# teshnizi/GraphEnvs

Measured on AMD Instinct MI355X. Metric: env-steps/sec (whole node), ShortestPath-v0 n=64 m=192 batch=65536, 1/2/4/8 GPU, higher is better.
Workload: dtype u64; 1 GPU; ShortestPath-v0 n_nodes=64 n_edges=192 weighted, 65536 env slots per GPU, random valid actions on device, same-step autoreset (seed-exact G(n,m)+features on device); envs_per_gpu=65536, prefetch_period=0, episodes_finished_per_gpu=6165512, settle_steps=128, parallelism=batch shard x1, no collective

## Files before the change

graphenvs_amd/csrc/ge_reset.h:

```cpp
#pragma once
#include "ge_params.h"
#include "ge_platform.h"

GE_DEV double ge_wlut(int code) {
  const int k = (code >= 3 && code <= 9) ? code : 10;
  return (double)k / 10.0;
}

GE_DEV uint32_t ge_temper(uint32_t y) {
  y ^= (y >> 11);
  y ^= (y << 7) & 0x9d2c5680u;
  y ^= (y << 15) & 0xefc60000u;
  y ^= (y >> 18);
  return y;
}

GE_DEV void ge_mt_twist(uint32_t *mt, int lane) {
  const int lo[3] = {0, GE_MT_N - GE_MT_M, 2 * (GE_MT_N - GE_MT_M)}, hi[3] = {GE_MT_N - GE_MT_M, 2 * (GE_MT_N - GE_MT_M), GE_MT_N};
#pragma unroll
  for (int ph = 0; ph < 3; ph++) {
    uint32_t a[4], b[4], c[4];
#pragma unroll
    for (int k = 0; k < 4; k++) {
      const int i = lo[ph] + lane + 64 * k;
// ... 89 lines not shown
  ge_wave_sync();
}


GE_DEV void ge_mt_load(uint32_t *mt, const uint32_t *src, int lane) {
  uint32_t r[10];
#pragma unroll
  for (int k = 0; k < 10; k++) { int i = lane + 64 * k; r[k] = i < GE_MT_N ? src[i] : 0u; }
#pragma unroll
  for (int k = 0; k < 10; k++) { int i = lane + 64 * k; if (i < GE_MT_N) mt[i] = r[k]; }
  ge_wave_sync();
}

GE_DEV void ge_mt_save(uint32_t *dst, const uint32_t *mt, int pos, int lane) {
  ge_wave_sync();
#pragma unroll
  for (int k = 0; k < 10; k++) { int i = lane + 64 * k; if (i < GE_MT_N) dst[i] = mt[i]; }
  if (lane == 0) dst[GE_MT_N] = (uint32_t)pos;
}

GE_DEV int ge_wave_incl_scan(int x, int lane) {
  for (int off = 1; off < GE_WAVE; off <<= 1) {
    int t = ge_shfl_i32(x, lane >= off ? lane - off : 0);
    if (lane >= off) x += t;
  }
  return x;
}

GE_DEV uint32_t ge_mask_below(uint32_t v) {
  return v ? (0xffffffffu >> ge_clz32(v)) : 0u;
}

struct GeRctx {
  uint32_t *mt, *mt2, *wm; uint64_t *abits; uint32_t *elist; int *fill; int *rowptr; uint16_t *colw; uint8_t *wsort;
  uint32_t *tmp; int *dist; int *perm;
  double *sigma, *delta;
  uint64_t *bits; int *misc;
};

GE_DEV GeRctx ge_carve(const GeParams &P) {
  unsigned char *s = ge_dyn_smem();
  const GeLds &L = P.lds;
  GeRctx c;
  c.mt = (uint32_t *)(s + L.mt); c.mt2 = (uint32_t *)(s + L.mt2); c.wm = (uint32_t *)(s + L.wm); c.abits = (uint64_t *)(s + L.abits); c.elist = (uint32_t *)(s + L.elist);
  c.fill = (int *)(s + L.fill); c.rowptr = (int *)(s + L.rowptr); c.colw = (uint16_t *)(s + L.colw);
  c.wsort = (uint8_t *)(s + L.wsort); c.tmp = (uint32_t *)(s + L.tmp); c.dist = (int *)(s + L.dist);
  c.perm = (int *)(s + L.perm);
  double *f = (double *)(s + L.f64a);
  c.sigma = f; c.delta = f + P.n;
  c.bits = (uint64_t *)(s + L.bits); c.misc = (int *)(s + L.misc);
  return c;
}

GE_DEV int ge_reach_wave(const GeRctx &c, int ng, int W, int start, const uint64_t *removed, int lane) {
  uint64_t *fr = c.bits, *vis = c.bits + W, *nx = c.bits + 2 * W;
  if (lane < W) {
    uint64_t s = ((start >> 6) == lane) ? (1ull << (start & 63)) : 0ull;
    fr[lane] = s; vis[lane] = s | (removed ? removed[lane] : 0ull);
  }
  ge_wave_sync();
  for (;;) {
    uint64_t any = 0;
    for (int k = 0; k < W; k++) {
      int v = k * GE_WAVE + lane;
      bool hit = false;
      if (v < ng && !((vis[k] >> lane) & 1ull)) {
        for (int w = 0; w < W; w++) if (c.abits[v * W + w] & fr[w]) { hit = true; break; }
      }
      uint64_t b = ge_ballot(hit);
      if (lane == 0) nx[k] = b;
      any |= b;
    }
    ge_wave_sync();
    if (!any) break;
    if (lane < W) { vis[lane] |= nx[lane]; fr[lane] = nx[lane]; }
    ge_wave_sync();
  }
  int cnt = 0;
  for (int w = 0; w < W; w++) cnt += ge_popc64(vis[w] & ~(removed ? removed[w] : 0ull));
  ge_wave_sync();
  return cnt;
}

GE_DEV bool ge_connected(const GeRctx &c, int ng, int W, int skip, int lane) {
  uint64_t *rem = c.bits + 3 * W;
  if (lane < W) rem[lane] = (skip >= 0 && (skip >> 6) == lane) ? (1ull << (skip & 63)) : 0ull;
  ge_wave_sync();
  int start = (skip == 0) ? 1 : 0;
  return ge_reach_wave(c, ng, W, start, rem, lane) == ng - (skip >= 0 ? 1 : 0);
}

GE_DEV double ge_pw_leaf(const double *a, int n, int lane) {
  if (n < 8) {
    double res = 0.0;
    for (int i = 0; i < n; i++) res += a[i];
    return res;
  }
  int lim = n - (n % 8);
  double r = 0.0;
  if (lane < 8) { r = a[lane]; for (int i = 8; i < lim; i += 8) r += a[i + lane]; }
  double r0 = ge_shfl_f64(r, 0), r1 = ge_shfl_f64(r, 1), r2 = ge_shfl_f64(r, 2), r3 = ge_shfl_f64(r, 3);
  double r4 = ge_shfl_f64(r, 4), r5 = ge_shfl_f64(r, 5), r6 = ge_shfl_f64(r, 6), r7 = ge_shfl_f64(r, 7);
  double res = ((r0 + r1) + (r2 + r3)) + ((r4 + r5) + (r6 + r7));
  for (int i = lim; i < n; i++) res += a[i];
  return res;
}
template <int D>
GE_DEV double ge_pw(const double *a, int n, int lane) {
  if (n <= 128) return ge_pw_leaf(a, n, lane);
  if constexpr (D > 0) {
    int n2 = n / 2; n2 -= n2 % 8;
    double l = ge_pw<D - 1>(a, n2, lane);
    double r = ge_pw<D - 1>(a + n2, n - n2, lane);
    return l + r;
  } else {
    return 0.0;
  }
}

GE_DEV int ge_rank_below(const uint64_t *row, int v) {
  int r = 0;
  for (int w = 0; w < (v >> 6); w++) r += ge_popc64(row[w]);
  return r + ge_popc64(row[v >> 6] & ((1ull << (v & 63)) - 1ull));
}

GE_DEV int ge_list_nbr(const GeParams &P, const GeRctx &c, int idx) {
  if (P.nocolw) { const int u = (int)(((uint64_t)(uint32_t)idx * P.div_m) >> 40), k = idx - u * (P.ng - 1); return k < u ? k : k + 1; }
  return (int)(c.colw[idx] >> 4);
}
GE_DEV int ge_list_code(const GeParams &P, const GeRctx &c, int idx) {
  if (P.nowsort) {
    if (!P.weighted) return 10;
    const int u = (int)(((uint64_t)(uint32_t)idx * P.div_m) >> 40), k = idx - u * (P.ng - 1), v = k < u ? k : k + 1;
    const int a = u < v ? u : v, b = u < v ? v : u;
    return (int)((const uint8_t *)c.wm)[a * (P.ng - 1) - ((a * (a - 1)) >> 1) + (b - a - 1)];
  }
  return P.nocolw ? (int)c.wsort[idx] : (int)(c.colw[idx] & 15);
}

GE_DEV int ge_row_of(const GeParams &P, const GeRctx &c, int idx) {
  return P.complete ? (int)(((uint64_t)(uint32_t)idx * P.div_m) >> 40) : (int)c.tmp[idx];
}

GE_DEV int ge_sorted_pos(const GeRctx &c, int W, int u, int v) { return c.rowptr[u] + ge_rank_below(c.abits + u * W, v); }
GE_DEV int ge_sorted_pos_p(const GeParams &P, const GeRctx &c, int u, int v) {
  return P.complete ? c.rowptr[u] + v - (v > u ? 1 : 0) : ge_sorted_pos(c, P.W, u, v);
}


struct GeInject { const int64_t *links; const uint8_t *wcode; const float *x; const int32_t *terminals; const uint32_t *seeds; };
#ifndef GE_GNM_ROUND_CAP
#define GE_GNM_ROUND_CAP (1 << 22)
#endif


#if defined(GE_STAMPS) && !defined(GE_EMU)
__device__ unsigned long long ge_stamp_buf[32];
#define GE_STAMP(k) do { if (lane == 0 && env == 0) { ge_stamp_buf[k] = wall_clock64(); if ((k) == 11) ge_stamp_buf[30] = clock64(); if ((k) == 17) ge_stamp_buf[31] = clock64(); } } while (0)
#define GE_STAMP_T0(k) do { if (tid == 0 && env == 0) ge_stamp_buf[k] = wall_clock64(); } while (0)
#define GE_STAMP_B0(k) do { if (lane == 0 && ge_bid() == 0) ge_stamp_buf[k] = wall_clock64(); } while (0)
#elif defined(GE_STAMP_SLOTS) && !defined(GE_EMU)
#define GE_STAMP(k) do { if (lane == 0) { if ((k) == 0) P.buf.final_cost[env] = (double)wall_clock64(); else if ((k) == 2) P.buf.final_len[env] = (int32_t)(wall_clock64() - (unsigned long long)P.buf.final_cost[env]); else if ((k) == 10) P.buf.final_heur[env] = (double)wall_clock64(); } } while (0)
#define GE_STAMP_T0(k) do { } while (0)
#define GE_STAMP_B0(k) do { } while (0)
#else
#define GE_STAMP(k) do { } while (0)
#define GE_STAMP_T0(k) do { } while (0)
#define GE_STAMP_B0(k) do { } while (0)
#endif


GE_DEV void ge_np_sink(const GeParams &P, const GeRctx &c, int sink, int idx, uint32_t val) {
  const int n = P.n, W = P.W;
  const uint32_t code = (sink == 3 ? 1u : 3u) + val;
  if (sink == 3) ((uint8_t *)c.wm)[P.cost_off + idx] = (uint8_t)code;
  else if (sink == 0) atomicOr(&c.wm[idx >> 3], code << (4 * (idx & 7)));
  else if (sink == 1) ((uint8_t *)c.wm)[idx] = (uint8_t)code;
  else {
    const int i = (int)((unsigned)idx / (unsigned)n), j = idx - i * n;
    if (i < j && ((c.abits[i * W + (j >> 6)] >> (j & 63)) & 1ull)) {
      c.wsort[ge_sorted_pos(c, W, i, j)] = (uint8_t)code; c.wsort[ge_sorted_pos(c, W, j, i)] = (uint8_t)code;
    }
  }
}

GE_DEV void ge_np_draws(const GeParams &P, const GeRctx &c, uint32_t *mt, int &nppos, int total, int lane, int sink) {
  int base = 0;
  const uint32_t bm = (sink == 3) ? 3u : 7u;
  const uint64_t below = (1ull << lane) - 1ull;
  while (base < total) {
    if (nppos >= GE_MT_N && total - base > GE_MT_N) {
      uint32_t R[GE_MT_ROWS];
      ge_mt_to_regs(R, mt, lane);
      do {
        ge_mt_twist_regs(R, lane);
#pragma unroll
        for (int k = 0; k < GE_MT_ROWS; k++) {
          const uint32_t val = (GE_WAVE * k + lane < GE_MT_N) ? (ge_temper(R[k]) & bm) : bm;
          const uint64_t bal = ge_ballot(val < bm);
          if (val < bm) ge_np_sink(P, c, sink, base + ge_popc64(bal & below), val);
          base += ge_popc64(bal);
        }
      } while (total - base > GE_MT_N);
      ge_mt_from_regs(mt, R, lane);
      ge_wave_sync();
      nppos = GE_MT_N;
      continue;
    }
    if (nppos >= GE_MT_N) { ge_mt_twist(mt, lane); nppos = 0; }
    if (GE_MT_N - nppos >= 4 * GE_WAVE) {
      uint32_t val[4]; uint64_t bal[4];
#pragma unroll
      for (int k = 0; k < 4; k++) val[k] = ge_temper(mt[nppos + GE_WAVE * k + lane]) & bm;
      int tot = 0;
#pragma unroll
      for (int k = 0; k < 4; k++) { bal[k] = ge_ballot(val[k] < bm); tot += ge_popc64(bal[k]); }
      if (base + tot < total) {
        int off = base;
#pragma unroll
        for (int k = 0; k < 4; k++) {
          if (val[k] < bm) ge_np_sink(P, c, sink, off + ge_popc64(bal[k] & below), val[k]);
          off += ge_popc64(bal[k]);
        }
        base = off; nppos += 4 * GE_WAVE;
        continue;
      }
    }
    {
      const int p = nppos + lane; const bool valid = p < GE_MT_N;
      const uint32_t val = valid ? (ge_temper(mt[p]) & bm) : 8u;
      const bool acc = valid && val < bm;
      const uint64_t bal = ge_ballot(acc);
      const int rank = ge_popc64(bal & below);
      const int idx = base + rank;
      if (acc && idx < total) ge_np_sink(P, c, sink, idx, val);
      const int nacc = ge_popc64(bal);
      if (base + nacc >= total) {
        const int need = total - base - 1;
        const uint64_t lastb = ge_ballot(acc && rank == need);
        nppos += ge_ctz64(lastb) + 1;
        base = total;
      } else {
        base += nacc;
        nppos += (GE_MT_N - nppos < GE_WAVE) ? (GE_MT_N - nppos) : GE_WAVE;
      }
    }
  }
  ge_wave_sync();
}

GE_DEV void ge_np_edge_cells(const GeParams &P, const GeRctx &c, uint32_t *tcell, int lane) {
  const int n = P.n, W = P.W;
  {
    int carry = 0;
    for (int k0 = 0; k0 < n; k0 += GE_WAVE) {
      const int u = k0 + lane; int d = 0;
      if (u < n) for (int w = u >> 6; w < W; w++) { uint64_t b = c.abits[u * W + w]; if (w == (u >> 6)) b &= ~((2ull << (u & 63)) - 1ull); d += ge_popc64(b); }
      const int incl = ge_wave_incl_scan(d, lane);
      if (u < n) c.dist[u] = carry + incl - d;
      carry += ge_shfl_i32(incl, GE_WAVE - 1);
    }
    ge_wave_sync();
    for (int u = lane; u < n; u += GE_WAVE) {
      int t = c.dist[u];
      for (int w = u >> 6; w < W; w++) {
        uint64_t b = c.abits[u * W + w]; if (w == (u >> 6)) b &= ~((2ull << (u & 63)) - 1ull);
        for (; b; b &= b - 1) tcell[t++] = (uint32_t)(u * n + w * 64 + ge_ctz64(b));
      }
    }
    ge_wave_sync();
  }
}
GE_DEV int ge_np_edge_number(const GeRctx &c, int W, int u, int v) {
  const int a = u < v ? u : v, b = u < v ? v : u;
  int t = c.dist[a];
  for (int w = a >> 6; w <= (b >> 6); w++) {
    uint64_t bits = c.abits[a * W + w];
    if (w == (a >> 6)) bits &= ~((2ull << (a & 63)) - 1ull);
    if (w == (b >> 6)) bits &= (1ull << (b & 63)) - 1ull;
    t += ge_popc64(bits);
  }
  return t;
}
GE_DEV void ge_np_draws_cells(const GeParams &P, const GeRctx &c, uint32_t *mt, int &nppos, int lane, const uint32_t *tcell, uint8_t *tcode) {
  const int n = P.n, m = P.m, total = n * n;
  const uint64_t below = (1ull << lane) - 1ull;
  GE_STAMP_B0(7);
  int base = 0, t = 0, t0 = 0;
  uint32_t treg = lane < m ? tcell[lane] : 0xffffffffu;
  uint32_t next = ge_readlane_u32(treg, 0);
  auto take = [&](uint32_t val, uint64_t bal, int cnt) {
    while (next - (uint32_t)base < (uint32_t)cnt) {
      const int r = (int)(next - (uint32_t)base);
      if (((bal >> lane) & 1ull) && ge_popc64(bal & below) == r) tcode[t] = (uint8_t)(3u + val);
      t++;
      if (t - t0 == GE_WAVE) { t0 = t; treg = (t0 + lane < m) ? tcell[t0 + lane] : 0xffffffffu; }
      next = ge_readlane_u32(treg, t - t0);
    }
  };
  while (base < total) {
    if (nppos >= GE_MT_N && total - base > GE_MT_N) {
      uint32_t R[GE_MT_ROWS];
      ge_mt_to_regs(R, mt, lane);
      do {
        ge_mt_twist_regs(R, lane);
        int tot = 0;
// ... 692 lines not shown
    if (path_like) {
      for (int i = lane; i < (n * n + 7) / 8; i += GE_WAVE) c.wm[i] = 0u;
      ge_wave_sync();
      ge_np_draws(P, c, c.mt2, nppos, n * n, lane, 0);
    } else ge_np_draws(P, c, c.mt2, nppos, t == GE_TSP ? P.m : n, lane, 1);
  }
  GE_STAMP(22);
  if (t == GE_DISTRIBUTION_CENTER) ge_np_draws(P, c, c.mt2, nppos, n, lane, 3);
  if (t == GE_PERISHABLE_DELIVERY) {
    const uint32_t ra = ge_np_next(c.mt2, nppos, lane), rb = ge_np_next(c.mt2, nppos, lane);
    if (lane == 0) { *(double *)c.misc = ((double)(int32_t)(ra >> 5) * 67108864.0 + (double)(int32_t)(rb >> 6)) / 9007199254740992.0; c.misc[2] = nppos; }
    ge_wave_sync();
    return;
  }
  if (t == GE_MULTICAST_ROUTING) ge_np_multicast_tail(P, c, c.mt2, nppos, lane);
  else if (path_like) ge_np_terminals(P, c, c.mt2, nppos, lane, n, P.T);
  GE_STAMP(23);
  if (save) ge_mt_save(save, c.mt2, nppos, lane);
}

template <class RP, class CW>
GE_DEV uint64_t ge_dc_search(double cutoff, int n, int s, const RP *rowptr, const CW *colw, double *S, int ss, uint8_t *stk, int ks) {
  (void)stk; (void)ks;
  for (int v = 0; v < n; v++) S[v * ss] = __builtin_inf();
  S[s * ss] = 0.0;
  uint64_t reached = 1ull << s, cur = 1ull << s;
  while (cur) {
    uint64_t nxt = 0;
    for (; cur; cur &= cur - 1) {
      const int u = ge_ctz64(cur);
      const double du = S[u * ss];
      const int r1 = rowptr[u + 1];
      for (int k0 = rowptr[u]; k0 < r1; k0 += 4) {
        uint32_t e[4]; double sv[4];
#pragma unroll
        for (int j = 0; j < 4; j++) e[j] = (uint32_t)colw[k0 + j < r1 ? k0 + j : k0];
#pragma unroll
        for (int j = 0; j < 4; j++) sv[j] = S[(int)(e[j] >> 4) * ss];
#pragma unroll
        for (int j = 0; j < 4; j++) {
          const int v = (int)(e[j] >> 4);
          const double d = du + ge_wlut((int)(e[j] & 15u));
          if (k0 + j < r1 && d <= cutoff && d < sv[j]) {
            S[v * ss] = d; reached |= 1ull << v;
            if (d + 0.3 <= cutoff) nxt |= 1ull << v;
          }
        }
      }
    }
    cur = nxt;
  }
  return reached;
}

template <int ENV>
GE_DEV void ge_write_edge_slabs(const GeParams &P, const GeRctx &c, int env, int tid, int nthreads) {
  constexpr int t = ENV;
  const ge_buffers &G = P.buf;
  const int n = P.n, W = P.W, E = P.E;
  const int64_t nbase = (int64_t)env * n, ebase = (int64_t)env * E, Ne = P.edge_row_stride;
  for (int idx = tid; idx < E; idx += nthreads) {
    int u = ge_row_of(P, c, idx), v = ge_list_nbr(P, c, idx), code = ge_list_code(P, c, idx);
    G.edge_index[ebase + idx] = P.node_id_base + nbase + u;
    G.edge_index[Ne + ebase + idx] = P.node_id_base + nbase + v;
    float wv = (t == GE_DENSEST_SUBGRAPH || t == GE_MAX_INDEPENDENT_SET) ? 1.f : (float)ge_wlut(code);
    if (P.spatial) wv = (float)G.sw64[ebase + ge_sorted_pos_p(P, c, u, v)];
    if (P.Fe == 2) { G.edge_attr[(ebase + idx) * 2] = wv; G.edge_attr[(ebase + idx) * 2 + 1] = 0.f; }
    else G.edge_attr[ebase + idx] = wv;
    G.colw[ebase + idx] = (uint16_t)((v << 4) | code);
    G.scode[ebase + idx] = P.nowsort ? (uint8_t)code : c.wsort[idx];
    if (G.rev_edge) {
      const int r0 = c.rowptr[v], r1 = c.rowptr[v + 1];
      int r = -1;
      for (int k0 = r0; k0 < r1 && r < 0; k0 += 4) {
        int w[4];
#pragma unroll
        for (int j = 0; j < 4; j++) w[j] = (int)(c.colw[k0 + j < r1 ? k0 + j : r0] >> 4);
#pragma unroll
        for (int j = 3; j >= 0; j--) if (k0 + j < r1 && w[j] == u) r = k0 + j;
      }
      G.rev_edge[ebase + idx] = r;
    }
  }
  for (int v = tid; v <= n; v += nthreads) G.row_ptr[(int64_t)env * (n + 1) + v] = c.rowptr[v];
  for (int i = tid; i < n * W; i += nthreads) G.adj_bits[nbase * W + i] = c.abits[i];
  if (G.node_rec) {
    for (int v = tid; v < n; v += nthreads) {
      uint64_t codes = 0; int d = c.rowptr[v + 1] - c.rowptr[v]; if (d > 16) d = 16;
      for (int k = 0; k < d; k++) codes |= (uint64_t)(c.wsort[c.rowptr[v] + k] & 15) << (4 * k);
      G.node_rec[(nbase + v) * 2] = c.abits[v]; G.node_rec[(nbase + v) * 2 + 1] = codes;
    }
  }
}

template <int ENV>
GE_DEV void ge_reset_env(const GeParams &P, int env, const uint32_t *seeds, const GeRun &run, const GeInject &inj) {
  const int tid = ge_tid_fresh();
  const int lane = tid & (GE_WAVE - 1);
  const int wv = tid >> 6;
  const int n = P.n, ng = P.ng, W = P.W, m = P.m, E = P.E, F = P.F, T = P.T;
  constexpr int t = ENV;
  const bool path_like_t = (t == GE_SHORTEST_PATH || t == GE_LONGEST_PATH || t == GE_STEINER_TREE || t == GE_MULTICAST_ROUTING);
  GeRctx c = ge_carve(P);
  const int64_t nbase = (int64_t)env * n, ebase = (int64_t)env * E;
  const bool restart = run.restart != 0;
  const bool next = run.next != 0;
  const bool queued = run.items == GE_ITEMS_QUEUE && !run.refill;
  const int64_t episode = restart ? 0 : P.buf.episode[env] + (next ? 1 : 0);
  const uint32_t seed = restart ? (run.restart == 1 ? seeds[env] : inj.seeds[env]) : P.buf.seed[env] + (next ? (uint32_t)P.seed_stride : 0u);
  const int ring = (int)(episode % GE_SEED_DEPTH);
  auto keep_at = [&](int which) -> uint32_t * { return P.buf.stream_state ? P.buf.stream_state + ((int64_t)env * 2 + which) * GE_STREAM_WORDS : nullptr; };
  auto pos0 = [&](int which) -> int { return run.cont ? (int)keep_at(which)[GE_MT_N] : GE_MT_N; };
  const uint32_t *mt_src = P.buf.mt_state + ((int64_t)env * GE_SEED_DEPTH + ring) * 2 * GE_MT_N;
  if (run.cont) mt_src = keep_at(0);
  int src = 0, dest = -1;
  int ppd_pk[5] = {-1, -1, -1, -1, -1}, ppd_dp[5] = {-1, -1, -1, -1, -1};
  bool gen_failed = false;
  double ppd_dt = 0.0;
  if (wv == 1) {
    if (!run.inject) { ge_numpy_wave<ENV>(P, c, run.cont ? keep_at(1) : mt_src + GE_MT_N, lane, env, pos0(1), keep_at(1)); ge_sync(); }
    ge_sync();
    ge_write_edge_slabs<ENV>(P, c, env, tid, 2 * GE_WAVE);
    ge_sync();
    return;
  }

  GE_STAMP(0);
  if (!run.inject) {
    ge_mt_load(c.mt, mt_src, lane);
    GE_STAMP(1);
    int pypos = pos0(0);
    int ppd_attempt = 0, ppd_pos = 0;
    bool failed = false;
    const int shift = 32 - (32 - ge_clz32((uint32_t)ng));
    for (;;) {
      GE_STAMP(29);
      for (int i = lane; i < n * W; i += GE_WAVE) c.abits[i] = 0ull;
      ge_wave_sync();
      if (P.complete) {
        for (int v = lane; v < ng; v += GE_WAVE)
          for (int w = 0; w < W; w++) {
            int lo = w * 64, hi = lo + 64; if (hi > ng) hi = ng;
            uint64_t bitsw = (hi <= lo) ? 0ull : ((hi - lo == 64) ? ~0ull : ((1ull << (hi - lo)) - 1ull));
            if ((v >> 6) == w) bitsw &= ~(1ull << (v & 63));
            c.abits[v * W + w] = bitsw;
          }
      } else {
        int cnt = 0, have_u = 0, carry_u = 0;
        const uint64_t below = (1ull << lane) - 1ull;
        int rounds = 0;
        for (;;) {
          if (++rounds > GE_GNM_ROUND_CAP) { failed = true; break; }
          if (pypos >= GE_MT_N) { ge_mt_twist(c.mt, lane); pypos = 0; }
          const int p0 = pypos + lane, p1 = p0 + GE_WAVE;
          const bool valid0 = p0 < GE_MT_N, valid1 = p1 < GE_MT_N;
          const uint32_t r0 = valid0 ? (ge_temper(c.mt[p0]) >> shift) : (uint32_t)ng, r1 = valid1 ? (ge_temper(c.mt[p1]) >> shift) : (uint32_t)ng;
          const bool pick0 = valid0 && r0 < (uint32_t)ng, pick1 = valid1 && r1 < (uint32_t)ng;
          const uint64_t V0 = ge_ballot(pick0), V1 = ge_ballot(pick1);
          const int n0 = ge_popc64(V0);
          const bool is_v0 = pick0 && ((ge_popc64(V0 & below) + have_u) & 1), is_v1 = pick1 && ((n0 + ge_popc64(V1 & below) + have_u) & 1);
          const uint64_t b0 = V0 & below, b1 = V1 & below;
          const uint32_t ur0 = ge_shfl_u32(r0, b0 ? 63 - (int)__builtin_clzll(b0) : 0), ur1 = ge_shfl_u32(r1, b1 ? 63 - (int)__builtin_clzll(b1) : 0);
          const int last0 = V0 ? (int)ge_readlane_u32(r0, 63 - (int)__builtin_clzll(V0)) : carry_u;
          const int u0 = b0 ? (int)ur0 : carry_u, v0 = (int)r0, u1 = b1 ? (int)ur1 : last0, v1 = (int)r1;
          const bool elig0 = is_v0 && u0 != v0 && !((c.abits[u0 * W + (v0 >> 6)] >> (v0 & 63)) & 1ull);
          const bool elig1 = is_v1 && u1 != v1 && !((c.abits[u1 * W + (v1 >> 6)] >> (v1 & 63)) & 1ull);
          const uint32_t key0 = elig0 ? (uint32_t)((u0 < v0 ? u0 : v0) << 12 | (u0 < v0 ? v0 : u0)) : 0xffffffffu;
          const uint32_t key1 = elig1 ? (uint32_t)((u1 < v1 ? u1 : v1) << 12 | (u1 < v1 ? v1 : u1)) : 0xfffffffeu;
          (void)ge_ballot(elig0 || elig1);
          bool lost0 = false, lost1 = false;
          if (elig0) {
            const int a = u0 < v0 ? u0 : v0, b = u0 < v0 ? v0 : u0; const unsigned long long bit = 1ull << (b & 63);
            lost0 = (atomicOr((unsigned long long *)&c.abits[a * W + (b >> 6)], bit) & bit) != 0;
          }
          if (elig1) {
            const int a = u1 < v1 ? u1 : v1, b = u1 < v1 ? v1 : u1; const unsigned long long bit = 1ull << (b & 63);
            lost1 = (atomicOr((unsigned long long *)&c.abits[a * W + (b >> 6)], bit) & bit) != 0;
          }
          bool dup0 = false, dup1 = false;
          uint64_t rem0 = ge_ballot(lost0), rem1 = ge_ballot(lost1);
          while (rem0 | rem1) {
            const uint32_t k0 = rem0 ? ge_readlane_u32(key0, ge_ctz64(rem0)) : ge_readlane_u32(key1, ge_ctz64(rem1));
            const uint64_t same0 = ge_ballot(elig0 && key0 == k0), same1 = ge_ballot(elig1 && key1 == k0);
            if (elig0 && key0 == k0 && lane != ge_ctz64(same0)) dup0 = true;
            if (elig1 && key1 == k0 && (same0 != 0ull || lane != ge_ctz64(same1))) dup1 = true;
            rem0 &= ~same0; rem1 &= ~same1;
          }
          bool acc0 = elig0 && !dup0, acc1 = elig1 && !dup1;
          const uint64_t A0 = ge_ballot(acc0), A1 = ge_ballot(acc1);
          const int na0 = ge_popc64(A0), na1 = ge_popc64(A1);
          const int arank0 = ge_popc64(A0 & below), arank1 = na0 + ge_popc64(A1 & below);
          const bool last_round = cnt + na0 + na1 >= m;
          int consumed, nacc = na0 + na1;
          if (last_round) {
            const int need = m - cnt - 1;
            bool undo0 = false, undo1 = false;
            if (need < na0) { const int fl = ge_ctz64(ge_ballot(acc0 && arank0 == need)); undo0 = acc0 && lane > fl; undo1 = acc1; acc0 = acc0 && lane <= fl; acc1 = false; consumed = fl + 1; }
            else { const int fl = ge_ctz64(ge_ballot(acc1 && arank1 == need)); undo1 = acc1 && lane > fl; acc1 = acc1 && lane <= fl; consumed = GE_WAVE + fl + 1; }
            if (undo0) { const int a = u0 < v0 ? u0 : v0, b = u0 < v0 ? v0 : u0; atomicAnd((unsigned long long *)&c.abits[a * W + (b >> 6)], ~(1ull << (b & 63))); }
            if (undo1) { const int a = u1 < v1 ? u1 : v1, b = u1 < v1 ? v1 : u1; atomicAnd((unsigned long long *)&c.abits[a * W + (b >> 6)], ~(1ull << (b & 63))); }
            nacc = need + 1;
          } else {
            consumed = (GE_MT_N - pypos < 2 * GE_WAVE) ? (GE_MT_N - pypos) : 2 * GE_WAVE;
            const int npick = n0 + ge_popc64(V1) + have_u;
            have_u = npick & 1;
            if (have_u && (V0 | V1)) carry_u = V1 ? (int)ge_readlane_u32(r1, 63 - (int)__builtin_clzll(V1)) : last0;
          }
          if (acc0) {
            atomicOr((unsigned long long *)&c.abits[u0 * W + (v0 >> 6)], (unsigned long long)(1ull << (v0 & 63)));
            atomicOr((unsigned long long *)&c.abits[v0 * W + (u0 >> 6)], (unsigned long long)(1ull << (u0 & 63)));
            c.elist[cnt + arank0] = (uint32_t)u0 | ((uint32_t)v0 << 16);
          }
          if (acc1) {
            atomicOr((unsigned long long *)&c.abits[u1 * W + (v1 >> 6)], (unsigned long long)(1ull << (v1 & 63)));
            atomicOr((unsigned long long *)&c.abits[v1 * W + (u1 >> 6)], (unsigned long long)(1ull << (u1 & 63)));
            c.elist[cnt + arank1] = (uint32_t)u1 | ((uint32_t)v1 << 16);
          }
          cnt += nacc; pypos += consumed;
          ge_wave_sync();
          if (last_round) break;
        }
      }
      ge_wave_sync();
      GE_STAMP(26);
      if (failed) break;
      uint64_t low = 0;
      for (int k = 0; k < W; k++) {
        const int v = k * GE_WAVE + lane; int d = 0;
        if (v < ng) for (int w = 0; w < W; w++) d += ge_popc64(c.abits[v * W + w]);
        low |= ge_ballot(v < ng && (d == 0 || (t == GE_TSP && d == 1)));
      }
      GE_STAMP(27);
      bool ok = !low && ge_connected(c, ng, W, -1, lane);
      GE_STAMP(28);
      if (ok && t == GE_TSP) ok = ge_connected(c, ng, W, 0, lane);
      if (ok && t == GE_PERISHABLE_DELIVERY) {
        double rnd;
        const bool late = P.weighted && !P.np_early;
        if (ppd_attempt == 0) { ge_sync(); if (late) ppd_pos = pos0(1); else { ppd_pos = c.misc[2]; rnd = *(const double *)c.misc; } }
        if (ppd_attempt > 0 || late) {
          if (late) { ge_np_edge_cells(P, c, c.tmp, lane); ge_np_draws_cells(P, c, c.mt2, ppd_pos, lane, c.tmp, (uint8_t *)c.wm); }
          else if (P.weighted) { for (int i = lane; i < (n * n + 7) / 8; i += GE_WAVE) c.wm[i] = 0u; ge_wave_sync(); ge_np_draws(P, c, c.mt2, ppd_pos, n * n, lane, 0); }
          const uint32_t ra = ge_np_next(c.mt2, ppd_pos, lane), rb = ge_np_next(c.mt2, ppd_pos, lane);
          rnd = ((double)(int32_t)(ra >> 5) * 67108864.0 + (double)(int32_t)(rb >> 6)) / 9007199254740992.0;
        }
        ppd_attempt++;
        ok = (n > GE_PPD_WIDE_ABOVE) ? ge_ppd_place_wide(P, c, rnd, ppd_pos, ppd_pk, ppd_dp, ppd_dt, lane)
                       : ge_ppd_place(P, c, (double *)(ge_dyn_smem() + P.lds.fw), rnd, ppd_pos, ppd_pk, ppd_dp, ppd_dt, lane);
      }
      if (ok) break;
      ge_wave_priority(1);
    }
    ge_wave_priority(0);
    if (failed) {
      if (lane == 0) atomicOr((unsigned int *)&P.buf.work_count[1], 1u);
      gen_failed = true;
      for (int i = lane; i < n * W; i += GE_WAVE) c.abits[i] = 0ull;
      ge_wave_sync();
      if (lane == 0) {
        int cnt = 0;
        for (int d = 1; d < ng && cnt < m; d++)
          for (int u = 0; u + d < ng && cnt < m; u++) {
            const int v = u + d;
            c.abits[u * W + (v >> 6)] |= 1ull << (v & 63); c.abits[v * W + (u >> 6)] |= 1ull << (u & 63);
            c.elist[cnt++] = (uint32_t)u | ((uint32_t)v << 16);
          }
      }
      ge_wave_sync();
      if (t == GE_PERISHABLE_DELIVERY) { if (ppd_attempt == 0) { ge_sync(); ppd_pos = c.misc[2]; } for (int i = 0; i < P.n_dests; i++) { ppd_pk[i] = i; ppd_dp[i] = P.n_dests + i; } }
    }
    if (P.buf.stream_state) {
      ge_mt_save(keep_at(0), c.mt, pypos, lane);
      if (t == GE_PERISHABLE_DELIVERY) ge_mt_save(keep_at(1), c.mt2, ppd_pos, lane);
    }
  } else {
    for (int i = lane; i < n * W; i += GE_WAVE) c.abits[i] = 0ull;
    for (int v = lane; v < n; v += GE_WAVE) c.fill[v] = 0;
    ge_wave_sync();
    for (int idx = lane; idx < E; idx += GE_WAVE) {
      int u = (int)inj.links[(ebase + idx) * 2], v = (int)inj.links[(ebase + idx) * 2 + 1];
      atomicAdd(&c.fill[u], 1);
      atomicOr((unsigned long long *)&c.abits[u * W + (v >> 6)], (unsigned long long)(1ull << (v & 63)));
    }
    ge_wave_sync();
  }

  GE_STAMP(2);
  if (!run.inject) {
    for (int v = lane; v < n; v += GE_WAVE) { int d = 0; for (int w = 0; w < W; w++) d += ge_popc64(c.abits[v * W + w]); c.fill[v] = d; }
    ge_wave_sync();
  }
  {
    int carry = 0;
    for (int k0 = 0; k0 < n; k0 += GE_WAVE) {
      int v = k0 + lane; int d = v < n ? c.fill[v] : 0;
      int incl = ge_wave_incl_scan(d, lane);
      if (v < n) c.rowptr[v] = carry + incl - d;
      carry += ge_shfl_i32(incl, GE_WAVE - 1);
    }
    if (lane == 0) c.rowptr[n] = carry;
    ge_wave_sync();
  }
  if (run.inject) {
    for (int idx = lane; idx < E; idx += GE_WAVE) {
      int u = (int)inj.links[(ebase + idx) * 2], v = (int)inj.links[(ebase + idx) * 2 + 1];
      c.colw[idx] = (uint16_t)((v << 4) | (inj.wcode[ebase + idx] & 15));
      if (!P.complete) c.tmp[idx] = (uint32_t)u;
    }
    ge_wave_sync();
  } else if (P.complete) {
    if (!P.nocolw) for (int idx = lane; idx < E; idx += GE_WAVE) {
      const int u = ge_row_of(P, c, idx), k = idx - u * (ng - 1);
      int v = k < u ? k : k + 1;
      c.colw[idx] = (uint16_t)((v << 4) | 10);
    }
    ge_wave_sync();
  } else {
    for (int v = lane; v < n; v += GE_WAVE) c.fill[v] = 0;
    ge_wave_sync();
    for (int id = lane; id < m; id += GE_WAVE) {
      uint32_t e = c.elist[id]; int u = (int)(e & 0xffffu), v = (int)(e >> 16);
      int s = c.rowptr[u] + atomicAdd(&c.fill[u], 1); c.tmp[s] = ((uint32_t)id << 16) | (uint32_t)v;
      int s2 = c.rowptr[v] + atomicAdd(&c.fill[v], 1); c.tmp[s2] = ((uint32_t)id << 16) | (uint32_t)u;
    }
    ge_wave_sync();
    for (int v = lane; v < n; v += GE_WAVE) {
      int lo = c.rowptr[v], hi = c.rowptr[v + 1];
      for (int a = lo + 1; a < hi; a++) {
        uint32_t key = c.tmp[a]; int b = a - 1;
        while (b >= lo && c.tmp[b] > key) { c.tmp[b + 1] = c.tmp[b]; b--; }
        c.tmp[b + 1] = key;
      }
    }
    ge_wave_sync();
    for (int idx = lane; idx < E; idx += GE_WAVE) c.colw[idx] = (uint16_t)(((c.tmp[idx] & 0xffffu) << 4) | 10u);
    ge_wave_sync();
    for (int v = lane; v < n; v += GE_WAVE) for (int k = c.rowptr[v]; k < c.rowptr[v + 1]; k++) c.tmp[k] = (uint32_t)v;
    ge_wave_sync();
  }

  GE_STAMP(3);
  if (!run.inject && t != GE_PERISHABLE_DELIVERY) ge_sync();
  if (!run.inject) {
    if (!P.nowsort) for (int idx = lane; idx < E; idx += GE_WAVE) c.wsort[idx] = 10;
    ge_wave_sync();
    const bool path_like = path_like_t;
    const bool matrix_w = path_like_t || t == GE_DISTRIBUTION_CENTER || t == GE_PERISHABLE_DELIVERY;
    if (P.weighted && matrix_w && P.np_early) {
      for (int idx = lane; idx < E; idx += GE_WAVE) {
        int u = ge_row_of(P, c, idx), v = c.colw[idx] >> 4;
        int a = u < v ? u : v, b = u < v ? v : u, cell = a * n + b;
        c.wsort[ge_sorted_pos_p(P, c, u, v)] = (uint8_t)((c.wm[cell >> 3] >> (4 * (cell & 7))) & 15u);
      }
    } else if (P.spatial) {
      const double *xy = (const double *)(c.wm + 4 * n);
      for (int idx = lane; idx < E; idx += GE_WAVE) {
        int u = ge_row_of(P, c, idx), v = c.colw[idx] >> 4;
        int a = u < v ? u : v, b = u < v ? v : u;
        double dx = xy[2 * a] - xy[2 * b], dy = xy[2 * a + 1] - xy[2 * b + 1];
        P.buf.sw64[ebase + ge_sorted_pos_p(P, c, u, v)] = __builtin_sqrt(dx * dx + dy * dy);
      }
    } else if (P.weighted && t == GE_TSP && P.complete) {
      if (!P.nowsort) for (int idx = lane; idx < E; idx += GE_WAVE) {
        const int u = ge_row_of(P, c, idx), v = ge_list_nbr(P, c, idx);
        const int a = u < v ? u : v, b = u < v ? v : u;
        c.wsort[ge_sorted_pos_p(P, c, u, v)] = ((const uint8_t *)c.wm)[a * (ng - 1) - ((a * (a - 1)) >> 1) + (b - a - 1)];
      }
    } else if (P.weighted && t == GE_TSP) {
      int carry = 0;
// ... 447 lines not shown
```

Measured before the change: 396.2 million env-steps/s.

## Compact picked MT samples into one pair per lane in G(n,m) edge sampling

The G(n,m) edge sampler now reads four wave-widths of Mersenne Twister output per round, ballots which samples fall in range, and compacts them so each lane handles one (u,v) pair, located through a popcount-based select64. Before, each lane tested two raw slots, and only about half the picked samples became the v of a pair. The goal is to fill the wave with candidate edges each round, so fewer rounds and fewer duplicate-resolution ballots are needed. The cost is extra select/popcount work and gathered mt reads per round, plus more intricate consumed/carry bookkeeping that must keep the seed-exact sequence.

```diff
diff --git a/graphenvs_amd/csrc/ge_reset.h b/graphenvs_amd/csrc/ge_reset.h
--- a/graphenvs_amd/csrc/ge_reset.h
+++ b/graphenvs_amd/csrc/ge_reset.h
@@ -265,6 +265,18 @@
 #ifndef GE_GNM_ROUND_CAP
 #define GE_GNM_ROUND_CAP (1 << 22)
 #endif
+
+GE_DEV int ge_select64(uint64_t x, int r) {
+  uint32_t w = (uint32_t)x;
+  int pos = 0, cnt = ge_popc64((uint64_t)w);
+  if (r >= cnt) { r -= cnt; pos = 32; w = (uint32_t)(x >> 32); }
+#pragma unroll
+  for (int s = 16; s; s >>= 1) {
+    cnt = ge_popc64((uint64_t)(w & ((1u << s) - 1u)));
+    if (r >= cnt) { r -= cnt; pos += s; w >>= s; }
+  }
+  return pos;
+}
 
 
 #if defined(GE_STAMPS) && !defined(GE_EMU)
@@ -1263,69 +1275,67 @@
         for (;;) {
           if (++rounds > GE_GNM_ROUND_CAP) { failed = true; break; }
           if (pypos >= GE_MT_N) { ge_mt_twist(c.mt, lane); pypos = 0; }
-          const int p0 = pypos + lane, p1 = p0 + GE_WAVE;
-          const bool valid0 = p0 < GE_MT_N, valid1 = p1 < GE_MT_N;
-          const uint32_t r0 = valid0 ? (ge_temper(c.mt[p0]) >> shift) : (uint32_t)ng, r1 = valid1 ? (ge_temper(c.mt[p1]) >> shift) : (uint32_t)ng;
-          const bool pick0 = valid0 && r0 < (uint32_t)ng, pick1 = valid1 && r1 < (uint32_t)ng;
-          const uint64_t V0 = ge_ballot(pick0), V1 = ge_ballot(pick1);
-          const int n0 = ge_popc64(V0);
-          const bool is_v0 = pick0 && ((ge_popc64(V0 & below) + have_u) & 1), is_v1 = pick1 && ((n0 + ge_popc64(V1 & below) + have_u) & 1);
-          const uint64_t b0 = V0 & below, b1 = V1 & below;
-          const uint32_t ur0 = ge_shfl_u32(r0, b0 ? 63 - (int)__builtin_clzll(b0) : 0), ur1 = ge_shfl_u32(r1, b1 ? 63 - (int)__builtin_clzll(b1) : 0);
-          const int last0 = V0 ? (int)ge_readlane_u32(r0, 63 - (int)__builtin_clzll(V0)) : carry_u;
-          const int u0 = b0 ? (int)ur0 : carry_u, v0 = (int)r0, u1 = b1 ? (int)ur1 : last0, v1 = (int)r1;
-          const bool elig0 = is_v0 && u0 != v0 && !((c.abits[u0 * W + (v0 >> 6)] >> (v0 & 63)) & 1ull);
-          const bool elig1 = is_v1 && u1 != v1 && !((c.abits[u1 * W + (v1 >> 6)] >> (v1 & 63)) & 1ull);
-          const uint32_t key0 = elig0 ? (uint32_t)((u0 < v0 ? u0 : v0) << 12 | (u0 < v0 ? v0 : u0)) : 0xffffffffu;
-          const uint32_t key1 = elig1 ? (uint32_t)((u1 < v1 ? u1 : v1) << 12 | (u1 < v1 ? v1 : u1)) : 0xfffffffeu;
-          (void)ge_ballot(elig0 || elig1);
-          bool lost0 = false, lost1 = false;
-          if (elig0) {
-            const int a = u0 < v0 ? u0 : v0, b = u0 < v0 ? v0 : u0; const unsigned long long bit = 1ull << (b & 63);
-            lost0 = (atomicOr((unsigned long long *)&c.abits[a * W + (b >> 6)], bit) & bit) != 0;
+          uint32_t raw[4];
+#pragma unroll
+          for (int j = 0; j < 4; j++) { const int p = pypos + j * GE_WAVE + lane; raw[j] = p < GE_MT_N ? c.mt[p] : 0xffffffffu; }
+          uint64_t V[4];
+#pragma unroll
+          for (int j = 0; j < 4; j++) V[j] = ge_ballot(pypos + j * GE_WAVE + lane < GE_MT_N && (ge_temper(raw[j]) >> shift) < (uint32_t)ng);
+          const int c0 = ge_popc64(V[0]), c1 = c0 + ge_popc64(V[1]), c2 = c1 + ge_popc64(V[2]), npick = c2 + ge_popc64(V[3]);
+          const int q1 = V[0] ? 63 - (int)__builtin_clzll(V[0]) : -1, q2 = V[1] ? 127 - (int)__builtin_clzll(V[1]) : q1;
+          const int q3 = V[2] ? 191 - (int)__builtin_clzll(V[2]) : q2, qlast = V[3] ? 255 - (int)__builtin_clzll(V[3]) : q3;
+          const int npk = npick + have_u;
+          const bool full = (npk >> 1) >= GE_WAVE;
+          const bool has = lane < (npk >> 1);
+          const int iv = 2 * lane + 1 - have_u;
+          const int j = (iv >= c0) + (iv >= c1) + (iv >= c2);
+          const uint64_t Vj = j == 0 ? V[0] : j == 1 ? V[1] : j == 2 ? V[2] : V[3];
+          const int vbit = ge_select64(Vj, iv - (j == 0 ? 0 : j == 1 ? c0 : j == 2 ? c1 : c2));
+          const uint64_t pm = Vj & ((1ull << vbit) - 1ull);
+          const int vpos = has ? j * GE_WAVE + vbit : 0;
+          const int upos = !has ? -1 : pm ? j * GE_WAVE + 63 - (int)__builtin_clzll(pm) : (j == 0 ? -1 : j == 1 ? q1 : j == 2 ? q2 : q3);
+          const uint32_t wv = c.mt[pypos + vpos], wu = c.mt[pypos + (upos < 0 ? 0 : upos)], wl = c.mt[pypos + (qlast < 0 ? 0 : qlast)];
+          const int v = has ? (int)(ge_temper(wv) >> shift) : 0;
+          const int u = !has ? 0 : upos < 0 ? carry_u : (int)(ge_temper(wu) >> shift);
+          const int a = u < v ? u : v, b = u < v ? v : u;
+          const unsigned long long bit = 1ull << (b & 63);
+          const bool elig = has && u != v && !((c.abits[u * W + (v >> 6)] >> (v & 63)) & 1ull);
+          const uint32_t key = elig ? (uint32_t)(a << 12 | b) : 0xffffffffu;
+          (void)ge_ballot(elig);
+          const bool lost = elig && (atomicOr((unsigned long long *)&c.abits[a * W + (b >> 6)], bit) & bit) != 0;
+          bool dup = false;
+          uint64_t rem = ge_ballot(lost);
+          while (rem) {
+            const uint32_t k0 = ge_readlane_u32(key, ge_ctz64(rem));
+            const uint64_t same = ge_ballot(elig && key == k0);
+            if (elig && key == k0 && lane != ge_ctz64(same)) dup = true;
+            rem &= ~same;
           }
-          if (elig1) {
-            const int a = u1 < v1 ? u1 : v1, b = u1 < v1 ? v1 : u1; const unsigned long long bit = 1ull << (b & 63);
-            lost1 = (atomicOr((unsigned long long *)&c.abits[a * W + (b >> 6)], bit) & bit) != 0;
-          }
-          bool dup0 = false, dup1 = false;
-          uint64_t rem0 = ge_ballot(lost0), rem1 = ge_ballot(lost1);
-          while (rem0 | rem1) {
-            const uint32_t k0 = rem0 ? ge_readlane_u32(key0, ge_ctz64(rem0)) : ge_readlane_u32(key1, ge_ctz64(rem1));
-            const uint64_t same0 = ge_ballot(elig0 && key0 == k0), same1 = ge_ballot(elig1 && key1 == k0);
-            if (elig0 && key0 == k0 && lane != ge_ctz64(same0)) dup0 = true;
-            if (elig1 && key1 == k0 && (same0 != 0ull || lane != ge_ctz64(same1))) dup1 = true;
-            rem0 &= ~same0; rem1 &= ~same1;
-          }
-          bool acc0 = elig0 && !dup0, acc1 = elig1 && !dup1;
-          const uint64_t A0 = ge_ballot(acc0), A1 = ge_ballot(acc1);
-          const int na0 = ge_popc64(A0), na1 = ge_popc64(A1);
-          const int arank0 = ge_popc64(A0 & below), arank1 = na0 + ge_popc64(A1 & below);
-          const bool last_round = cnt + na0 + na1 >= m;
-          int consumed, nacc = na0 + na1;
+          bool acc = elig && !dup;
+          const uint64_t A = ge_ballot(acc);
+          const int arank = ge_popc64(A & below);
+          int nacc = ge_popc64(A);
+          const bool last_round = cnt + nacc >= m;
+          int consumed;
           if (last_round) {
             const int need = m - cnt - 1;
-            bool undo0 = false, undo1 = false;
-            if (need < na0) { const int fl = ge_ctz64(ge_ballot(acc0 && arank0 == need)); undo0 = acc0 && lane > fl; undo1 = acc1; acc0 = acc0 && lane <= fl; acc1 = false; consumed = fl + 1; }
-            else { const int fl = ge_ctz64(ge_ballot(acc1 && arank1 == need)); undo1 = acc1 && lane > fl; acc1 = acc1 && lane <= fl; consumed = GE_WAVE + fl + 1; }
-            if (undo0) { const int a = u0 < v0 ? u0 : v0, b = u0 < v0 ? v0 : u0; atomicAnd((unsigned long long *)&c.abits[a * W + (b >> 6)], ~(1ull << (b & 63))); }
-            if (undo1) { const int a = u1 < v1 ? u1 : v1, b = u1 < v1 ? v1 : u1; atomicAnd((unsigned long long *)&c.abits[a * W + (b >> 6)], ~(1ull << (b & 63))); }
+            const int fl = ge_ctz64(ge_ballot(acc && arank == need));
+            if (acc && lane > fl) atomicAnd((unsigned long long *)&c.abits[a * W + (b >> 6)], ~bit);
+            acc = acc && lane <= fl;
+            consumed = (int)ge_readlane_u32((uint32_t)vpos, fl) + 1;
             nacc = need + 1;
+          } else if (full) {
+            consumed = (int)ge_readlane_u32((uint32_t)vpos, GE_WAVE - 1) + 1;
+            have_u = 0;
           } else {
-            consumed = (GE_MT_N - pypos < 2 * GE_WAVE) ? (GE_MT_N - pypos) : 2 * GE_WAVE;
-            const int npick = n0 + ge_popc64(V1) + have_u;
-            have_u = npick & 1;
-            if (have_u && (V0 | V1)) carry_u = V1 ? (int)ge_readlane_u32(r1, 63 - (int)__builtin_clzll(V1)) : last0;
+            consumed = (GE_MT_N - pypos < 4 * GE_WAVE) ? (GE_MT_N - pypos) : 4 * GE_WAVE;
+            have_u = npk & 1;
+            if (have_u && npick) carry_u = (int)(ge_temper(wl) >> shift);
           }
-          if (acc0) {
-            atomicOr((unsigned long long *)&c.abits[u0 * W + (v0 >> 6)], (unsigned long long)(1ull << (v0 & 63)));
-            atomicOr((unsigned long long *)&c.abits[v0 * W + (u0 >> 6)], (unsigned long long)(1ull << (u0 & 63)));
-            c.elist[cnt + arank0] = (uint32_t)u0 | ((uint32_t)v0 << 16);
-          }
-          if (acc1) {
-            atomicOr((unsigned long long *)&c.abits[u1 * W + (v1 >> 6)], (unsigned long long)(1ull << (v1 & 63)));
-            atomicOr((unsigned long long *)&c.abits[v1 * W + (u1 >> 6)], (unsigned long long)(1ull << (u1 & 63)));
-            c.elist[cnt + arank1] = (uint32_t)u1 | ((uint32_t)v1 << 16);
+          if (acc) {
+            atomicOr((unsigned long long *)&c.abits[u * W + (v >> 6)], (unsigned long long)(1ull << (v & 63)));
+            atomicOr((unsigned long long *)&c.abits[v * W + (u >> 6)], (unsigned long long)(1ull << (u & 63)));
+            c.elist[cnt + arank] = (uint32_t)u | ((uint32_t)v << 16);
           }
           cnt += nacc; pypos += consumed;
           ge_wave_sync();
```

After: 395.2 million env-steps/s. No clear change (-0.3%).
